# oscarkey/safe-exploration

Hardware: AMD Instinct MI355X
Metric: cem_particle_step_evals_per_s (higher is better)
Workload: dtype f64

## Files before the change

### include/sx_amd.h

```cpp
#ifndef SX_AMD_H
#define SX_AMD_H

#include <stdint.h>

#ifdef __cplusplus
extern "C" {
#endif

#define SX_MAX_NS 4
#define SX_MAX_NU 2
#define SX_MAX_D (SX_MAX_NS + SX_MAX_NU)
#define SX_MAX_M 16
#define SX_TILE 16

#define SX_OK 0
#define SX_ERR_ARG 1
#define SX_ERR_UNSUPPORTED 2
#define SX_ERR_LAUNCH 3

#define SX_STATUS_NAN 1
#define SX_STATUS_ZERO_FIX 2
#define SX_STATUS_UB_NONPOS 4

#define SX_OBJ_NEG_VARIANCE 0
#define SX_OBJ_AFFINE_ABS 1
#define SX_CON_TERMINAL 0
#define SX_CON_ALL_STATES 1

#define SX_ACTION_VIOLATION_COST 3.0
#define SX_STATE_VIOLATION_COST 10.0

typedef struct sx_gp_model {
    int32_t n_s, n_u;
    int32_t n_train;
    int32_t n_pad;
    double inv_ls2[SX_MAX_NS * SX_MAX_D];
    double outputscale[SX_MAX_NS];
    double noise[SX_MAX_NS];
    const double* x_train;
    const double* a_pack;
    const int32_t* stage_tab;
} sx_gp_model;

typedef struct sx_env {
    int32_t n_s, n_u;
    int32_t m;
    int32_t obj_mode;
    int32_t con_mode;
    int32_t reserved;
    double beta;
    double a[SX_MAX_NS * SX_MAX_NS];
    double b[SX_MAX_NS * SX_MAX_NU];
    double k_fb[SX_MAX_NU * SX_MAX_NS];
    double l_mu[SX_MAX_NS];
    double l_sigma[SX_MAX_NS];
    double h_mat[SX_MAX_M * SX_MAX_NS];
    double h_vec[SX_MAX_M];
    double u_min[SX_MAX_NU];
    double u_max[SX_MAX_NU];
    double obj_w_abs[SX_MAX_NS];
    double obj_target[SX_MAX_NS];
    double obj_w_lin[SX_MAX_NS];
} sx_env;

const char* sx_version(void);

#define SX_FEAT_MAX_WIDTH 32
#define SX_FEAT_MAX_LAYERS 3
typedef struct sx_feat_model {
    int32_t n_s, n_u;
    int32_t n_feat;
    int32_t n_layers;
    int32_t normalise;
    int32_t width[SX_FEAT_MAX_LAYERS + 1];
    double prelu;
// ... 174 lines not shown
```

### safe_exploration_amd/csrc/sx_rollout_rh.hpp

```cpp
#pragma once
#include <hip/hip_runtime.h>

#include "../../include/sx_amd.h"
#include "sx_rollout_rw.hpp"

#ifndef SX_RH_REGP
#define SX_RH_REGP 26
#endif
#ifndef SX_RH_LEAD
#define SX_RH_LEAD -1
#endif
#ifndef SX_RH_LDSP
#define SX_RH_LDSP 8
#endif
#ifndef SX_RH_PFG
#define SX_RH_PFG 6
#endif
#ifndef SX_RH_PFL
#define SX_RH_PFL 2
#endif
#ifndef SX_RH_RBMAJOR
#define SX_RH_RBMAJOR 1
#endif
#ifndef SX_RH_PRIO
#define SX_RH_PRIO 0
#endif
#ifndef SX_RH_WFIRST
#define SX_RH_WFIRST 0
#endif
#ifndef SX_RH_SHARES
#define SX_RH_SHARES 4, 4, 4, 1, 4, 4, 4
#endif

namespace sx {

constexpr int kRhWaves = 8;
constexpr int kRhThreads = 64 * kRhWaves;

template <int NS, int NRB>
struct RhPlan {
    int wave_of[NS][NRB];
    int pairs[kRhWaves];
    constexpr RhPlan() : wave_of{}, pairs{} {
        for (int w = 0; w < kRhWaves; ++w) pairs[w] = 0;
        for (int d = 0; d < NS; ++d) {
            int lo = 0, n = kRhWaves;
            if (kRhWaves % NS == 0) {
                n = kRhWaves / NS;
                lo = d * n;
            }
            const bool rev = (kRhWaves % NS == 0) && (d & 1);
            int set_of[NRB] = {};
            int load[kRhWaves] = {};
            for (int rb = NRB - 1; rb >= 0; --rb) {
                int best = 0;
                for (int s = 1; s < n; ++s)
                    if (load[s] + pairs[lo + (rev ? n - 1 - s : s)] < load[best] + pairs[lo + (rev ? n - 1 - best : best)]) best = s;
                set_of[rb] = best;
                load[best] += 2 * (rb + 1);
            }
            for (int rb = 0; rb < NRB; ++rb) wave_of[d][rb] = lo + (rev ? n - 1 - set_of[rb] : set_of[rb]);
            for (int s = 0; s < n; ++s) pairs[lo + (rev ? n - 1 - s : s)] += load[s];
        }
    }
    constexpr int max_pairs() const {
        int m = 0;
        for (int w = 0; w < kRhWaves; ++w) m = pairs[w] > m ? pairs[w] : m;
        return m;
    }
    constexpr bool has(int w, int d) const {
        for (int rb = 0; rb < NRB; ++rb)
            if (wave_of[d][rb] == w) return true;
        return false;
    }
    constexpr int qmax(int w, int d) const {
        for (int rb = NRB - 1; rb >= 0; --rb)
            if (wave_of[d][rb] == w) return 2 * (rb + 1);
        return 0;
    }
};

template <int NS, int NRB>
struct RhElements {
    static constexpr int kMax = NS * NRB * (NRB + 1);
    short d[kRhWaves][kMax], rb[kRhWaves][kMax], q[kRhWaves][kMax];
    int n[kRhWaves];
    constexpr RhElements() : d{}, rb{}, q{}, n{} {
        const RhPlan<NS, NRB> plan{};
        for (int w = 0; w < kRhWaves; ++w) {
            int idx = 0;
            for (int dd = 0; dd < NS; ++dd) {
#if SX_RH_RBMAJOR
                for (int r = NRB - 1; r >= 0; --r)
                    for (int qq = 0; qq < 2 * (r + 1); ++qq)
                        if (plan.wave_of[dd][r] == w) { d[w][idx] = dd; rb[w][idx] = r; q[w][idx] = qq; ++idx; }
#else
                for (int qq = 0; qq < 2 * NRB; ++qq)
                    for (int r = NRB - 1; r >= 0; --r)
                        if (plan.wave_of[dd][r] == w && qq < 2 * (r + 1)) { d[w][idx] = dd; rb[w][idx] = r; q[w][idx] = qq; ++idx; }
#endif
            }
            n[w] = idx;
        }
    }
};

struct RhLayout {
    int nr, nl, ng, lead;
    constexpr RhLayout(int total, int regp, int ldsp)
        : nr(total < regp ? total : regp), nl(0), ng(0), lead(0) {
        nl = total - nr < ldsp ? total - nr : ldsp;
        ng = total - nr - nl;
        lead = SX_RH_LEAD < 0 || ng == 0 ? nr : (SX_RH_LEAD < nr ? SX_RH_LEAD : nr);
    }
    constexpr int storage(int e, int regp, int ldsp) const {
        if (SX_RH_LEAD < 0 || ng == 0) return e;
        if (e < lead) return e;
        if (e < lead + ng) return regp + ldsp + (e - lead);
        if (e < lead + ng + nl) return regp + (e - lead - ng);
        return lead + (e - lead - ng - nl);
    }
};

template <int NS, int NRB, int MAXP, int REGP, int LDSP>
struct RhStream {
    int pair[kRhWaves][MAXP];
    constexpr RhStream() : pair{} {
        const RhElements<NS, NRB> el{};
        constexpr int wpo = NRB * (NRB + 1);
        for (int w = 0; w < kRhWaves; ++w) {
            const RhLayout lay(el.n[w], REGP, LDSP);
            for (int i = 0; i < MAXP; ++i) pair[w][i] = 0;
            for (int e = 0; e < el.n[w]; ++e)
                pair[w][lay.storage(e, REGP, LDSP)] = el.d[w][e] * wpo + el.rb[w][e] * (el.rb[w][e] + 1) + el.q[w][e];
        }
    }
};

enum RhOpKind { kRhLoadB = 0, kRhLoadWL = 1, kRhLoadWG = 2, kRhMfma = 3, kRhRowEpi = 4, kRhFinalEpi = 5 };
struct RhOp {
    int kind;
    int i;
    int rb;
    int q;
    int d;
    int slot;
    int e;
};
template <int NS, int NRB, int WAVE, int REGP, int LDSP, int PF, int PFL, int PFG>
struct RhProgram {
    static constexpr int kMaxOps = 4 * NS * NRB * (NRB + 1) / 2 + 8 * NRB * NS + 16;
    RhOp ops[kMaxOps];
    int n;
    int total;
    constexpr RhProgram() : ops{}, n(0), total(0) {
        const RhElements<NS, NRB> el{};
        total = el.n[WAVE];
        const RhLayout lay(total, REGP, LDSP);
        int next_l = 0;
        int next_g = 0;
        const int e_g0 = (SX_RH_LEAD < 0 || lay.ng == 0) ? lay.nr + lay.nl : lay.lead;
        const int e_l0 = (SX_RH_LEAD < 0 || lay.ng == 0) ? lay.nr : lay.lead + lay.ng;
        int bslot[RhElements<NS, NRB>::kMax] = {};
        int bfirst[RhElements<NS, NRB>::kMax] = {};
        int nloads = 0;
        for (int e = 0; e < total; ++e) {
            const bool fresh = SX_RH_RBMAJOR || e == 0 || el.q[WAVE][e] != el.q[WAVE][e - 1] || el.d[WAVE][e] != el.d[WAVE][e - 1];
            if (fresh) ++nloads;
            bfirst[e] = fresh ? 1 : 0;
            bslot[e] = (nloads - 1) % (PF + 1);
        }
        constexpr int kDelay = 2;
        int pend_rb[NRB * NS] = {}, pend_d[NRB * NS] = {}, pend_at[NRB * NS] = {};
        int npend = 0, done = 0;
        int issued_b = 0;
        int eb = 0;
        auto issue_b_upto = [&](int loads_wanted) {
            while (issued_b < loads_wanted && eb < total) {
                if (bfirst[eb]) {
                    ops[n++] = RhOp{kRhLoadB, 0, 0, el.q[WAVE][eb], el.d[WAVE][eb], bslot[eb]};
                    ++issued_b;
                }
                ++eb;
            }
        };
        int loads_seen = 0;
        for (int e = 0; e < total; ++e) {
            if (bfirst[e]) ++loads_seen;
            issue_b_upto(loads_seen + PF);
            while (next_l < lay.nl && e_l0 + next_l <= e + PFL) ops[n++] = RhOp{kRhLoadWL, REGP + next_l++, 0, 0, 0, 0};
            while (next_g < lay.ng && e_g0 + next_g <= e + PFG) ops[n++] = RhOp{kRhLoadWG, REGP + LDSP + next_g++, 0, 0, 0, 0};
            ops[n++] = RhOp{kRhMfma, lay.storage(e, REGP, LDSP), el.rb[WAVE][e], el.q[WAVE][e], el.d[WAVE][e], bslot[e], e};
            const bool last_of_rb = el.q[WAVE][e] == 2 * (el.rb[WAVE][e] + 1) - 1;
            if (last_of_rb) {
                pend_rb[npend] = el.rb[WAVE][e];
                pend_d[npend] = el.d[WAVE][e];
                pend_at[npend] = e + kDelay;
                ++npend;
            }
            while (done < npend && pend_at[done] <= e) {
                ops[n++] = RhOp{kRhRowEpi, 0, pend_rb[done], 0, pend_d[done], 0};
                ++done;
            }
        }
        while (done < npend) {
            ops[n++] = RhOp{kRhRowEpi, 0, pend_rb[done], 0, pend_d[done], 0};
            ++done;
        }
        const RhPlan<NS, NRB> plan{};
        for (int d = 0; d < NS; ++d)
            if (plan.has(WAVE, d)) ops[n++] = RhOp{kRhFinalEpi, 0, 0, 0, d, 0};
    }
};

template <int NS, int D, int NRB, int WAVE, int REGP, int LDSP>
__device__ __forceinline__ void rh_mfma_phase(const GpConst<NS, D>& gc, GpTileLds<NS, D>& lds, const v2d* wlds_wave, int lane,
                                              const v2d (&wreg)[REGP]) {
    constexpr int PF = SX_RW_PF, PFL = SX_RH_PFL, PFG = SX_RH_PFG;
    constexpr int MAXP = RhPlan<NS, NRB>{}.max_pairs();
    static constexpr RhProgram<NS, NRB, WAVE, REGP, LDSP, PF, PFL, PFG> prog{};
    static constexpr RhStream<NS, NRB, MAXP, REGP, LDSP> stream{};
    const v2d* kbase = reinterpret_cast<const v2d*>(lds.kfrag) + lane;
    typedef const __attribute__((address_space(1))) v2d* gv2d;
    typedef const __attribute__((address_space(3))) v2d* lv2d;
    const v2d* ap_opaque = reinterpret_cast<const v2d*>(gc.a_pack) + lane;
    asm volatile("" : "+v"(ap_opaque));
    const gv2d ap = (gv2d)ap_opaque;
    const lv2d wl_base = (lv2d)wlds_wave + lane;
    v4d acc[NRB];
    v2d b[PF + 1];
    v2d wl[PFL + 1];
    v2d wg[PFG + 1];
    double ssq[NS];
#pragma unroll
    for (int d = 0; d < NS; ++d) ssq[d] = 0.0;
    static_for<0, prog.n>([&](auto ktag) {
        constexpr RhOp op = prog.ops[decltype(ktag)::value];
        if constexpr (op.kind == kRhLoadB) {
            b[op.slot] = kbase[(op.q * NS + op.d) * 64];
        } else if constexpr (op.kind == kRhLoadWL) {
            wl[op.i % (PFL + 1)] = wl_base[(op.i - REGP) * 64];
        } else if constexpr (op.kind == kRhLoadWG) {
            wg[op.i % (PFG + 1)] = ap[(size_t)stream.pair[WAVE][op.i] * 64];
        } else if constexpr (op.kind == kRhMfma) {
#if SX_RH_PRIO == 2
            if constexpr ((4 * op.e) / prog.total != (4 * (op.e - 1)) / prog.total || op.e == 0)
                __builtin_amdgcn_s_setprio(3 - (4 * op.e) / prog.total);
#endif
            SX_PIN();
            const v2d bq = b[op.slot];
            v2d a;
            if constexpr (op.i < REGP)
                a = wreg[op.i];
            else if constexpr (op.i < REGP + LDSP)
                a = wl[op.i % (PFL + 1)];
            else
                a = wg[op.i % (PFG + 1)];
            if constexpr (op.q == 0)
                acc[op.rb] = __builtin_amdgcn_mfma_f64_16x16x4f64(a.x, bq.x, v4d{0.0, 0.0, 0.0, 0.0}, 0, 0, 0);
            else
                acc[op.rb] = __builtin_amdgcn_mfma_f64_16x16x4f64(a.x, bq.x, acc[op.rb], 0, 0, 0);
            acc[op.rb] = __builtin_amdgcn_mfma_f64_16x16x4f64(a.y, bq.y, acc[op.rb], 0, 0, 0);
            SX_PIN();
        } else if constexpr (op.kind == kRhRowEpi) {
            constexpr int rb = op.rb, d = op.d;
            double s;
            if constexpr (rb >= NRB - 2) {
                const int row0 = rb * 16 + (lane >> 4);
                s = 0.0;
#pragma unroll
                for (int r = 0; r < 4; ++r) {
                    const int row = row0 + 4 * r;
                    if (row < gc.n_train)
                        s = fma(acc[rb][r], acc[rb][r], s);
                    else if (row - gc.n_train <= D)
                        lds.mj[d * 256 + (row - gc.n_train) * 16 + (lane & 15)] = acc[rb][r];
                }
            } else {
                s = fma(acc[rb][3], acc[rb][3], fma(acc[rb][2], acc[rb][2], fma(acc[rb][1], acc[rb][1], acc[rb][0] * acc[rb][0])));
            }
            ssq[d] += s;
        } else {
            constexpr int d = op.d;
            const v4d tot = __builtin_amdgcn_mfma_f64_16x16x4f64(1.0, ssq[d], v4d{0.0, 0.0, 0.0, 0.0}, 0, 0, 0);
            if (lane < 16) lds.part[(WAVE * NS + d) * 16 + lane] = tot[0];
        }
    });
}

template <int NS, int D, int NRB, bool WITH_JAC, typename G>
__device__ __forceinline__ void rh_collect(const G& gc, const GpTileLds<NS, D>& lds, int c, const double (&z)[D],
                                           double (&mean)[NS], double (&var)[NS], double (&jac)[NS][D]) {
    constexpr RhPlan<NS, NRB> plan{};
#pragma unroll
    for (int d = 0; d < NS; ++d) {
        double q = 0.0;
#pragma unroll
        for (int w = 0; w < kRhWaves; ++w)
            if (plan.has(w, d)) q += lds.part[(w * NS + d) * 16 + c];
        var[d] = (gc.outputscale[d] - q) + gc.noise[d];
        const double m = lds.mj[d * 256 + c];
        mean[d] = m;
        if constexpr (WITH_JAC) {
#pragma unroll
            for (int j = 0; j < D; ++j) jac[d][j] = lds.mj[d * 256 + (1 + j) * 16 + c] - z[j] * gc.inv_ls2[d * D + j] * m;
        }
    }
}

template <int NS, int NRB>
constexpr int rh_regp() {
    constexpr int m = RhPlan<NS, NRB>{}.max_pairs();
    return m < SX_RH_REGP ? m : SX_RH_REGP;
}
template <int NS, int NRB>
constexpr int rh_ldsp() {
    constexpr int rest = RhPlan<NS, NRB>{}.max_pairs() - rh_regp<NS, NRB>();
    return rest < SX_RH_LDSP ? rest : SX_RH_LDSP;
}
template <int NS, int NU, int NRB>
inline size_t rh_lds_doubles(int n_train, int n_pad, int H) {
    constexpr int D = NS + NU, S = NS + NS * NS;
    return (size_t)NS * n_pad * 16 + NS * 256 + (size_t)kRhWaves * NS * 16 + 32 * D + (((size_t)SX_TILE * H * NU + 1) & ~(size_t)1) +
           (((size_t)SX_TILE * (2 * (S + NS) + 3) + 1) & ~(size_t)1) + RwKstarLds<NS, D>::doubles(n_pad) +
           (size_t)kRhWaves * rh_ldsp<NS, NRB>() * 128;
}

template <int NS, int NU, int NRB>
__global__ __launch_bounds__(kRhThreads) void cem_rollout_rh_kernel(GpConst<NS, NS + NU> gc, ReachConst<NS, NU> rc,
                                                                    CostConst<SX_MAX_M, NS, NU> cc, RolloutPtrs rp) {
    constexpr int D = NS + NU;
    constexpr int S = NS + NS * NS;
    constexpr int PQS = S + NS;
    constexpr RhPlan<NS, NRB> plan{};
    constexpr int MAXP = plan.max_pairs();
    constexpr int REGP = rh_regp<NS, NRB>();
    constexpr int LDSP = rh_ldsp<NS, NRB>();
    extern __shared__ __attribute__((aligned(16))) double smem[];
    GpTileLds<NS, D> lds;
    constexpr int nw = kRhWaves;
    lds.xs = nullptr;
    lds.etab = nullptr;
    lds.kfrag = smem;
    lds.mj = lds.kfrag + (size_t)NS * gc.n_pad * 16;
    lds.part = lds.mj + NS * 256;
    lds.zs = lds.part + (size_t)nw * NS * 16;
    double* acts = lds.zs + 32 * D;
    const int tid = threadIdx.x;
    const int wave = __builtin_amdgcn_readfirstlane(tid >> 6), lane = tid & 63;
    const int H = rp.H;
    const int tiles_per_problem = (rp.P + SX_TILE - 1) / SX_TILE;
    const int total_tiles = rp.E * tiles_per_problem;

    RwConst<NS, NU>* const cst = reinterpret_cast<RwConst<NS, NU>*>(acts + (((size_t)SX_TILE * rp.H * NU + 1) & ~(size_t)1));
    double* const pq = reinterpret_cast<double*>(cst + 1);
    RwKstarLds<NS, D> kl;
    kl.carve(pq + (((size_t)SX_TILE * (2 * PQS + 3) + 1) & ~(size_t)1), gc.n_pad);
    v2d* const wlds = reinterpret_cast<v2d*>(kl.xbar + ((D + 1) & ~1));

    static constexpr RhStream<NS, NRB, MAXP, REGP, LDSP> stream{};
    v2d wreg[REGP];
#if SX_RH_WFIRST
    {
        const v2d* __restrict__ const ap0 = reinterpret_cast<const v2d*>(gc.a_pack) + lane;
#pragma unroll
        for (int i = 0; i < REGP; ++i) wreg[i] = ap0[(size_t)stream.pair[wave][i] * 64];
        if constexpr (LDSP > 0) {
#pragma unroll
            for (int i = 0; i < LDSP; ++i) wlds[(wave * LDSP + i) * 64 + lane] = ap0[(size_t)stream.pair[wave][REGP + i] * 64];
        }
    }
#endif
    {
        static_assert(sizeof(RwConst<NS, NU>) % 8 == 0 && sizeof(ReachConst<NS, NU>) % 8 == 0 &&
                      sizeof(CostConst<SX_MAX_M, NS, NU>) % 8 == 0, "copied in 8-byte words");
        constexpr int nrc = sizeof(ReachConst<NS, NU>) / 8, ncc = sizeof(CostConst<SX_MAX_M, NS, NU>) / 8;
        double* dst = reinterpret_cast<double*>(cst);
        const double* src_rc = reinterpret_cast<const double*>(&rc);
        const double* src_cc = reinterpret_cast<const double*>(&cc);
        for (int i = tid; i < nrc; i += kRhThreads) dst[i] = src_rc[i];
        for (int i = tid; i < ncc; i += kRhThreads) dst[nrc + i] = src_cc[i];
        if (tid < NS * D) cst->inv_ls2[tid] = gc.inv_ls2[tid];
        if (tid < NS) {
            cst->outputscale[tid] = gc.outputscale[tid];
            cst->noise[tid] = gc.noise[tid];
        }
    }
    const RwConst<NS, NU>& fc = *cst;
    const ReachConst<NS, NU>& frc = cst->rc;
    const CostConst<SX_MAX_M, NS, NU>& fcc = cst->cc;
    rw_kstar_setup(gc, kl, lds.kfrag);
    const int kstar_pairs = (gc.n_train + 7) >> 3;

    const bool owner = tid < SX_TILE;
    int q0_begin, q0_end, q_begin = 0, q_end = 0;
    kstar_pair_range(kstar_pairs, wave, 1, nw, q0_begin, q0_end);
    if (wave > 0) {
        constexpr int kShare[8] = {0, SX_RH_SHARES};
        int before = 0, total = 0;
#pragma unroll
        for (int w = 1; w < 8; ++w) {
            if (w < wave) before += kShare[w];
            total += kShare[w];
        }
        kstar_pair_range(kstar_pairs, before, kShare[wave], total, q_begin, q_end);
    }
    double* const zs_base = lds.zs;

    for (int tile = blockIdx.x; tile < total_tiles; tile += gridDim.x) {
#ifdef SX_STAMPS
        const unsigned long long tile_t0 = stamp();
        unsigned long long first_k = 0, first_kb = 0;
#endif
        const int e = tile / tiles_per_problem;
        const int c0 = (tile - e * tiles_per_problem) * SX_TILE;
        const bool valid = owner && (c0 + tid < rp.P);

        const double* dist_mean = rp.mean + (int64_t)e * H * NU;
        const double* dist_std = rp.std + (int64_t)e * H * NU;
        bool have_q = rp.q0 != nullptr;
        if (rp.elite_rows) {
            const int L = H * NU, W = 2 + L;
            double* const ms = lds.kfrag;
            const double* rows = rp.elite_rows + (int64_t)e * rp.elite_k * W + 2;
            const bool publish = c0 == 0 && rp.mean_out;
// ... 8 lines not shown
                    ms[col] = m;
                    ms[L + col] = sd;
                    if (publish) {
                        rp.mean_out[(int64_t)e * L + col] = m;
                        rp.std_out[(int64_t)e * L + col] = sd;
                    }
                }
            }
            __syncthreads();
            dist_mean = ms;
            dist_std = ms + L;
        }
        for (int i = tid; i < SX_TILE * H * NU; i += kRhThreads) {
            const int c = i / (H * NU);
            const int r = i - c * (H * NU);
            double a = 0.0;
            if (c0 + c < rp.P) {
                const int64_t gi = ((int64_t)e * rp.P + c0 + c) * (H * NU) + r;
                if (rp.noise) {
                    a = dist_mean[r] + dist_std[r] * rp.noise[gi];
                    rp.actions[gi] = a;
                } else {
                    a = rp.actions[gi];
                }
            }
            acts[i] = a;
        }
        const bool lane_owner = lane < SX_TILE;
        const bool lane_valid = lane_owner && (c0 + lane < rp.P);
        auto st_row = [&](int buf, int c) { return pq + (buf * SX_TILE + c) * PQS; };
        double* const ac_row = pq + 2 * SX_TILE * PQS + (lane_owner ? lane : 0) * 3;
        if (owner) {
            double* my = st_row(0, tid);
#pragma unroll
            for (int i = 0; i < NS; ++i) {
                my[i] = rp.x0[(int64_t)e * NS + i];
#pragma unroll
                for (int j = 0; j < NS; ++j) my[NS + i * NS + j] = have_q ? rp.q0[((int64_t)e * NS + i) * NS + j] : 0.0;
            }
            ac_row[0] = 0.0;
            ac_row[1] = 0.0;
            reinterpret_cast<int*>(ac_row + 2)[0] = 0;
        }
        __syncthreads();
        if (owner) {
            const double* my = st_row(0, tid);
#pragma unroll
            for (int i = 0; i < NS; ++i) lds.zs[tid * D + i] = my[i];
#pragma unroll
            for (int cidx = 0; cidx < NU; ++cidx) lds.zs[tid * D + NS + cidx] = acts[(tid * H + 0) * NU + cidx];
        }
        __syncthreads();

        if (!SX_RH_WFIRST && tile == (int)blockIdx.x) {
            const v2d* __restrict__ const ap = reinterpret_cast<const v2d*>(gc.a_pack) + lane;
            if constexpr (LDSP > 0) {
                const __amdgpu_buffer_rsrc_t arsrc =
                    __builtin_amdgcn_make_buffer_rsrc(const_cast<double*>(gc.a_pack), 0, (int)0xffffffffu, 0x00020000);
#pragma unroll
                for (int i = 0; i < LDSP; ++i) {
                    const int pair = __builtin_amdgcn_readfirstlane(stream.pair[wave][REGP + i]);
                    __builtin_amdgcn_raw_ptr_buffer_load_lds(
                        arsrc, (__attribute__((address_space(3))) void*)(wlds + (wave * LDSP + i) * 64), 16, lane * 16, pair << 10, 0, 0);
                }
            }
#pragma unroll
            for (int i = 0; i < REGP; ++i) wreg[i] = ap[(size_t)stream.pair[wave][i] * 64];
        }

        auto next_centre = [&](const ReachConst<NS, NU>& R, int c, const double* z_prev, double (&out)[NS]) {
#pragma unroll
            for (int i = 0; i < NS; ++i) {
                double s = lds.mj[i * 256 + c];
#pragma unroll
                for (int j = 0; j < NS; ++j) s = fma(R.a[i * NS + j], z_prev[j], s);
#pragma unroll
                for (int cidx = 0; cidx < NU; ++cidx) s = fma(R.b[i * NU + cidx], z_prev[NS + cidx], s);
                out[i] = s;
            }
        };
        auto finish_state = [&](int t) {
            double z[D], u[NU], mean[NS], var[NS], jac[NS][D], p1[NS], Q1[NS][NS];
            double p[NS], Q[NS][NS];
            constexpr RhPlan<NS, NRB> plan{};
            const double* my = st_row(t & 1, lane);
            double partv[NS][kRhWaves], mjv[NS][1 + D], ils2[NS][D], osc[NS], nzv[NS];
#pragma unroll
            for (int d = 0; d < NS; ++d) {
#pragma unroll
                for (int w = 0; w < kRhWaves; ++w) partv[d][w] = plan.has(w, d) ? lds.part[(w * NS + d) * 16 + lane] : 0.0;
#pragma unroll
                for (int r = 0; r < 1 + D; ++r) mjv[d][r] = lds.mj[d * 256 + r * 16 + lane];
            }
#pragma unroll
            for (int i = 0; i < NS; ++i) {
                p[i] = my[i];
#pragma unroll
                for (int j = 0; j < NS; ++j) Q[i][j] = my[NS + i * NS + j];
            }
#pragma unroll
            for (int cidx = 0; cidx < NU; ++cidx) u[cidx] = acts[(lane * H + t) * NU + cidx];
#pragma unroll
            for (int d = 0; d < NS; ++d) {
                osc[d] = fc.outputscale[d];
                nzv[d] = fc.noise[d];
#pragma unroll
                for (int j = 0; j < D; ++j) ils2[d][j] = fc.inv_ls2[d * D + j];
// ... 101 lines not shown
                    }
                    const double dist = hc + sqrt(hq) - hv;
                    viol = viol || (dist >= 0.0);
                }
            }
            unsigned long long bits = __ballot(viol);
            bits |= bits >> 32;
            bits |= bits >> 16;
            if (lane_owner) {
                if ((bits >> lane) & 1ull) con += SX_STATE_VIOLATION_COST;
                bool uviol = false;
#pragma unroll
                for (int cidx = 0; cidx < NU; ++cidx) uviol = uviol || (uu[cidx] < umin[cidx]) || (uu[cidx] > umax[cidx]);
                if (uviol) con += SX_ACTION_VIOLATION_COST;
                double oadd = 0.0;
                if (obj_mode == SX_OBJ_NEG_VARIANCE) {
#pragma unroll
                    for (int i = 0; i < NS; ++i) oadd -= var[i];
                } else {
#pragma unroll
                    for (int i = 0; i < NS; ++i) oadd += wab[i] * fabs(tgt[i] - pp[i]) + wli[i] * pp[i];
                }
                obj += oadd;
                ac_row[0] = obj;
                ac_row[1] = con;
                const int64_t g = (int64_t)e * rp.P + c0 + lane;
                if (lane_valid && rp.traj) {
                    double* tr = rp.traj + (g * H + t) * S;
#pragma unroll
                    for (int i = 0; i < NS; ++i) {
                        tr[i] = pp[i];
#pragma unroll
                        for (int j = 0; j < NS; ++j) tr[NS + i * NS + j] = QQ[i][j];
                    }
                }
                if (lane_valid && rp.sigma) {
#pragma unroll
                    for (int i = 0; i < NS; ++i) rp.sigma[(g * H + t) * NS + i] = var[i];
                }
            }
        };

#ifdef SX_STAMPS
        unsigned long long c_k = 0, c_kb = 0, c_m = 0, c_mb = 0;
        unsigned long long rt0;
        asm volatile("s_memrealtime %0\n\ts_waitcnt lgkmcnt(0)" : "=s"(rt0)::"memory");
        const unsigned long long ct0 = stamp();
#endif
        for (int t = 0; t < H; ++t) {
#ifdef SX_STAMPS
            const unsigned long long t0 = stamp();
#endif
            const bool kstar_wave = !(t > 0 && wave == 0);
            if (wave == 4 && t > 1) finish_costs(t - 2);
            if (kstar_wave) {
                double zq[D];
                const int c = lane & 15;
                if (t == 0) {
#pragma unroll
                    for (int j = 0; j < D; ++j) zq[j] = zs_base[c * D + j];
                    rw_kstar_phase(gc, kl, lds.kfrag, q0_begin, q0_end, zq);
                } else {
                    double pc[NS];
                    next_centre(rc, c, zs_base + ((t - 1) & 1) * 16 * D + c * D, pc);
#pragma unroll
                    for (int i = 0; i < NS; ++i) zq[i] = pc[i];
#pragma unroll
                    for (int cidx = 0; cidx < NU; ++cidx) zq[NS + cidx] = acts[(c * H + t) * NU + cidx];
                    rw_kstar_phase(gc, kl, lds.kfrag, q_begin, q_end, zq);
                }
            } else if (owner) {
                finish_state(t - 1);
            }
#ifdef SX_STAMPS
            const unsigned long long t1 = stamp();
#endif
            if (t == 0) asm volatile("s_waitcnt vmcnt(0)" ::: "memory");
            __syncthreads();
#ifdef SX_STAMPS
            const unsigned long long t2 = stamp();
#endif
            const v2d* wl = wlds + wave * LDSP * 64;
#if SX_RH_PRIO == 1
            if (wave < 4) __builtin_amdgcn_s_setprio(3);
#endif
            switch (wave) {
                case 0: rh_mfma_phase<NS, D, NRB, 0, REGP, LDSP>(gc, lds, wl, lane, wreg); break;
                case 1: rh_mfma_phase<NS, D, NRB, 1, REGP, LDSP>(gc, lds, wl, lane, wreg); break;
                case 2: rh_mfma_phase<NS, D, NRB, 2, REGP, LDSP>(gc, lds, wl, lane, wreg); break;
                case 3: rh_mfma_phase<NS, D, NRB, 3, REGP, LDSP>(gc, lds, wl, lane, wreg); break;
                case 4: rh_mfma_phase<NS, D, NRB, 4, REGP, LDSP>(gc, lds, wl, lane, wreg); break;
                case 5: rh_mfma_phase<NS, D, NRB, 5, REGP, LDSP>(gc, lds, wl, lane, wreg); break;
                case 6: rh_mfma_phase<NS, D, NRB, 6, REGP, LDSP>(gc, lds, wl, lane, wreg); break;
                default: rh_mfma_phase<NS, D, NRB, 7, REGP, LDSP>(gc, lds, wl, lane, wreg); break;
            }
#if SX_RH_PRIO == 1
            if (wave < 4) __builtin_amdgcn_s_setprio(0);
#elif SX_RH_PRIO == 2
            __builtin_amdgcn_s_setprio(0);
#endif
#ifdef SX_STAMPS
            const unsigned long long t3 = stamp();
#endif
            __syncthreads();
#ifdef SX_STAMPS
            const unsigned long long t4 = stamp();
            c_k += t1 - t0; c_kb += t2 - t1; c_m += t3 - t2; c_mb += t4 - t3;
            if (t == 0) { first_k = t1 - t0; first_kb = t2 - t1; }
#endif
        }
#ifdef SX_STAMPS
        const unsigned long long loop_t1 = stamp();
        if (rp.stamps && lane == 0 && tile == (int)blockIdx.x) {
            unsigned long long* o = rp.stamps + ((size_t)blockIdx.x * nw + wave) * 8;
            o[0] = c_k; o[1] = c_kb; o[2] = c_m; o[3] = c_mb;
            o[4] = (ct0 - tile_t0) | (first_k << 32);
            unsigned long long rt1;
            asm volatile("s_memrealtime %0\n\ts_waitcnt lgkmcnt(0)" : "=s"(rt1)::"memory");
            o[6] = stamp() - ct0;
            o[7] = rt1 - rt0;
        }
#endif
        if (wave == 0 && owner) finish_state(H - 1);
        if (wave == 4 && H > 1) finish_costs(H - 2);
        __syncthreads();
        if (wave == 0) finish_costs(H - 1);
        if (valid) {
            const int64_t g = (int64_t)e * rp.P + c0 + tid;
            rp.obj_cost[g] = ac_row[0];
            rp.con_cost[g] = ac_row[1];
            const int st = reinterpret_cast<const int*>(ac_row + 2)[0];
            if (st) atomicOr(rp.status, st);
        }
        __syncthreads();
#ifdef SX_STAMPS
        if (rp.stamps && lane == 0 && tile == (int)blockIdx.x)
            rp.stamps[((size_t)blockIdx.x * nw + wave) * 8 + 5] = (stamp() - loop_t1) | (first_kb << 32);
#endif
    }
}

}
```

### safe_exploration_amd/csrc/sx_rollout_rw.hpp

```cpp
#pragma once
#include <hip/hip_runtime.h>

#include "../../include/sx_amd.h"
#include "sx_exp2_tab2048.hpp"
#include "sx_gp.hpp"
#include "sx_reach.hpp"
#include "sx_refit.hpp"
#include "sx_rollout.hpp"
#include "sx_rw_launch.hpp"

#ifndef SX_RW_LDSCONST
#define SX_RW_LDSCONST 1
#endif
#ifndef SX_RW_POLYLANES
#define SX_RW_POLYLANES 1
#endif
#ifndef SX_RW_PF
#define SX_RW_PF 2
#endif
#ifndef SX_RW_RCLOCAL
#define SX_RW_RCLOCAL 0
#endif
#ifndef SX_RW_POLYFOLD
#define SX_RW_POLYFOLD 0
// ... 146 lines not shown
        if (lane < 16) lds.part[(WAVE * NS + d) * 16 + lane] = tot[0];
        }
    });
}

constexpr double kExpScale2 = 2048.0 / 0.693147180559945309417232;
constexpr double kExpUnit2 = 0.693147180559945309417232 / 2048.0;

template <int NS, int D>
struct RwKstarLds {
    double* rows;
    double* tab;
    double* xbar;
    static __host__ __device__ size_t doubles(int n_pad) { return (size_t)n_pad * (D + NS) + (n_pad & 1) + kExpTab2 + 2 + ((D + 1) & ~1); }
    __device__ void carve(double* base, int n_pad) {
        rows = base;
        tab = rows + (size_t)n_pad * (D + NS) + (n_pad & 1);
        xbar = tab + kExpTab2 + 2;
    }
};

template <int NS, int D>
__device__ __forceinline__ void rw_kstar_setup(const GpConst<NS, D>& gc, const RwKstarLds<NS, D>& kl, double* kfrag) {
    const int tid = threadIdx.x, lane = tid & 63;
    double xb[D];
#pragma unroll
    for (int j = 0; j < D; ++j) {
        double v = lane < gc.n_train ? gc.x_train[lane * D + j] : 0.0;
        for (int off = 32; off > 0; off >>= 1) v += __shfl_xor(v, off);
        xb[j] = v / (double)(gc.n_train < 64 ? gc.n_train : 64);
        if (tid == 0) kl.xbar[j] = xb[j];
    }
    for (int k = tid; k < gc.n_pad; k += blockDim.x) {
        double xr[D], cc[NS];
#pragma unroll
        for (int d = 0; d < NS; ++d) cc[d] = 0.0;
#pragma unroll
        for (int j = 0; j < D; ++j) {
            xr[j] = k < gc.n_train ? gc.x_train[k * D + j] - xb[j] : 0.0;
#pragma unroll
            for (int d = 0; d < NS; ++d) cc[d] = fma(gc.k_nh_ils2[d * D + j], xr[j] * xr[j], cc[d]);
        }
#pragma unroll
        for (int j = 0; j < D; ++j) kl.rows[k * (D + NS) + j] = xr[j];
#pragma unroll
        for (int d = 0; d < NS; ++d) kl.rows[k * (D + NS) + D + d] = cc[d];
    }
    for (int i = tid; i < kExpTab2; i += blockDim.x) kl.tab[i] = kExp2Tab2048[i];
    if (tid < 2) kl.tab[kExpTab2 + tid] = __builtin_nan("");
    const int first_pad = ((gc.n_train + 7) >> 3) * NS * 128;
    for (int i = first_pad + tid; i < (gc.n_pad >> 3) * NS * 128; i += blockDim.x) kfrag[i] = 0.0;
}

template <int NS, int D>
__device__ __forceinline__ void rw_kstar_phase(const GpConst<NS, D>& gc, const RwKstarLds<NS, D>& kl, double* kfrag,
                                               int q_begin, int q_end, const double (&z)[D]) {
    constexpr int M = 2 * NS, RS = D + NS;
    const int n = q_end - q_begin;
    if (n <= 0) return;
    const int lane = (int)threadIdx.x & 63;
    const int c = lane & 15;
    double zz[NS], g[NS][D];
    bool znan = false;
    {
        double zc[D];
#pragma unroll
        for (int j = 0; j < D; ++j) {
            zc[j] = z[j] - kl.xbar[j];
            znan = znan || (z[j] != z[j]);
        }
#pragma unroll
        for (int d = 0; d < NS; ++d) {
            double a = gc.k_log_os[d];
#pragma unroll
            for (int j = 0; j < D; ++j) {
                const double kz = gc.k_nh_ils2[d * D + j] * zc[j];
                a = fma(kz, zc[j], a);
                g[d][j] = -2.0 * kz;
            }
            zz[d] = a;
        }
    }
    const lds_f64* etab = (const lds_f64*)kl.tab + (znan ? kExpTab2 : 0);
    const int emask = znan ? 0 : kExpTab2 - 1;
    const int k0 = 8 * q_begin + (lane >> 4);
    const lds_f64* x = (const lds_f64*)kl.rows + k0 * RS;
    lds_f64* f = (lds_f64*)kfrag + kfrag_index(NS, c, k0, 0);

    struct Set {
        double t[M], p[M];
        int mi[M];
    };
    auto load_x = [&](double (&xx)[2 * RS]) {
        asm volatile("" : "+v"(x));
#pragma unroll
        for (int h = 0; h < 2; ++h)
#pragma unroll
            for (int j = 0; j < RS; ++j) xx[h * RS + j] = x[h * 4 * RS + j];
        x += 8 * RS;
    };
    auto stage_a1 = [&](const double (&xx)[2 * RS], Set& s) {
        double yc[M], m[M];
#pragma unroll
        for (int h = 0; h < 2; ++h)
#pragma unroll
            for (int d = 0; d < NS; ++d) {
                double a = xx[h * RS + D + d] + zz[d];
#pragma unroll
                for (int j = 0; j < D; ++j) a = fma(g[d][j], xx[h * RS + j], a);
                yc[h * NS + d] = a;
            }
#pragma unroll
        for (int i = 0; i < M; ++i) yc[i] = __builtin_fmax(yc[i], -800.0 * kExpScale2);
#pragma unroll
        for (int i = 0; i < M; ++i) m[i] = __builtin_rint(yc[i]);
#pragma unroll
        for (int i = 0; i < M; ++i) asm("v_cvt_i32_f64 %0, %1" : "=v"(s.mi[i]) : "v"(m[i]));
#pragma unroll
        for (int i = 0; i < M; ++i) s.t[i] = etab[s.mi[i] & emask];
#pragma unroll
#if SX_RW_POLYFOLD
        for (int i = 0; i < M; ++i) s.p[i] = yc[i] - m[i];
#else
        for (int i = 0; i < M; ++i) s.p[i] = (yc[i] - m[i]) * kExpUnit2;
#endif
    };
    auto stage_a2 = [&](Set& s) {
        double r[M];
#pragma unroll
        for (int i = 0; i < M; ++i) r[i] = s.p[i];
#pragma unroll
#if SX_RW_POLYFOLD
        for (int i = 0; i < M; ++i) s.p[i] = fma(r[i], kExpUnit2 * kExpUnit2 * kExpUnit2 / 6.0, kExpUnit2 * kExpUnit2 * 0.5);
#pragma unroll
        for (int i = 0; i < M; ++i) s.p[i] = fma(s.p[i], r[i], kExpUnit2);
#else
        for (int i = 0; i < M; ++i) s.p[i] = fma(r[i], 1.66666666666666666667e-01, 0.5);
#pragma unroll
        for (int i = 0; i < M; ++i) s.p[i] = fma(s.p[i], r[i], 1.0);
#endif
#pragma unroll
        for (int i = 0; i < M; ++i) s.p[i] = s.p[i] * r[i];
    };
    auto stage_b = [&](const Set& s) {
        asm volatile("" : "+v"(f));
        double val[M];
#pragma unroll
        for (int i = 0; i < M; ++i) val[i] = ldexp(fma(s.t[i], s.p[i], s.t[i]), s.mi[i] >> 11);
#pragma unroll
        for (int d = 0; d < NS; ++d) {
            f[d * 128] = val[d];
            f[d * 128 + 1] = val[NS + d];
        }
        f += NS * 128;
    };
    double xr[2 * RS];
    Set s0, s1;
    load_x(xr);
    stage_a1(xr, s0);
    load_x(xr);
    stage_a2(s0);
    auto body = [&](const Set& sold, Set& snew) {
        stage_a1(xr, snew);
        SX_PIN();
        load_x(xr);
        stage_b(sold);
        SX_PIN();
        stage_a2(snew);
        SX_PIN();
    };
    const int n1 = n - 1;
    for (int k = 0; k < (n1 >> 1); ++k) {
        body(s0, s1);
        body(s1, s0);
    }
    if (n1 & 1) {
        body(s0, s1);
        stage_b(s1);
    } else {
        stage_b(s0);
    }
}

template <int NS, int NU>
struct alignas(16) RwConst {
    ReachConst<NS, NU> rc;
    CostConst<SX_MAX_M, NS, NU> cc;
    double inv_ls2[NS * (NS + NU)];
    double outputscale[NS];
    double noise[NS];
};

template <int NS, int D, int NRB, bool WITH_JAC, typename G>
__device__ __forceinline__ void rw_collect(const G& gc, const GpTileLds<NS, D>& lds, int c,
                                           const double (&z)[D], double (&mean)[NS], double (&var)[NS],
                                           double (&jac)[NS][D]) {
    constexpr RwPlan<NS, NRB> plan{};
#pragma unroll
    for (int d = 0; d < NS; ++d) {
        double q = 0.0;
#pragma unroll
        for (int w = 0; w < kRwWaves; ++w)
            if (plan.has(w, d)) q += lds.part[(w * NS + d) * 16 + c];
        var[d] = (gc.outputscale[d] - q) + gc.noise[d];
        const double m = lds.mj[d * 256 + c];
        mean[d] = m;
        if constexpr (WITH_JAC) {
#pragma unroll
            for (int j = 0; j < D; ++j) jac[d][j] = lds.mj[d * 256 + (1 + j) * 16 + c] - z[j] * gc.inv_ls2[d * D + j] * m;
        }
    }
}

template <int NS, int NU, int NRB>
__global__ __launch_bounds__(kRwThreads) __attribute__((amdgpu_waves_per_eu(1, 1)))
void cem_rollout_rw_kernel(GpConst<NS, NS + NU> gc, ReachConst<NS, NU> rc, CostConst<SX_MAX_M, NS, NU> cc, RolloutPtrs rp) {
    constexpr int D = NS + NU;
    constexpr int S = NS + NS * NS;
    constexpr int PQS = S + 3;
    constexpr RwPlan<NS, NRB> plan{};
    constexpr int MAXP = plan.max_pairs();
    static_assert(MAXP <= kRwMaxPairs, "W does not fit the register budget");
    extern __shared__ __attribute__((aligned(16))) double smem[];
    GpTileLds<NS, D> lds;
    constexpr int nw = kRwWaves;
    double* acts = lds.carve(smem, gc.n_train, gc.n_pad, nw, NS);
    const int tid = threadIdx.x;
#if SX_RW_LDSCONST
    RwConst<NS, NU>* const cst = reinterpret_cast<RwConst<NS, NU>*>(acts + (((size_t)SX_TILE * rp.H * NU + 1) & ~(size_t)1));
    {
        static_assert(sizeof(RwConst<NS, NU>) % 8 == 0 && sizeof(ReachConst<NS, NU>) % 8 == 0 &&
                      sizeof(CostConst<SX_MAX_M, NS, NU>) % 8 == 0, "copied in 8-byte words");
        constexpr int nrc = sizeof(ReachConst<NS, NU>) / 8, ncc = sizeof(CostConst<SX_MAX_M, NS, NU>) / 8;
        double* dst = reinterpret_cast<double*>(cst);
// ... 331 lines not shown
```

Measured before the change: 465.3 million.

## Replace block barrier with LDS generation-flag handoff between Kstar and MFMA waves

Result: slower. 429.8 million (-7.6%).

```diff
diff --git a/include/sx_amd.h b/include/sx_amd.h
--- a/include/sx_amd.h
+++ b/include/sx_amd.h
@@ -21,6 +21,7 @@
 #define SX_STATUS_NAN 1
 #define SX_STATUS_ZERO_FIX 2
 #define SX_STATUS_UB_NONPOS 4
+#define SX_STATUS_HANDOFF_TIMEOUT 32
 
 #define SX_OBJ_NEG_VARIANCE 0
 #define SX_OBJ_AFFINE_ABS 1
diff --git a/safe_exploration_amd/csrc/sx_rollout_rh.hpp b/safe_exploration_amd/csrc/sx_rollout_rh.hpp
--- a/safe_exploration_amd/csrc/sx_rollout_rh.hpp
+++ b/safe_exploration_amd/csrc/sx_rollout_rh.hpp
@@ -4,12 +4,6 @@
 #include "../../include/sx_amd.h"
 #include "sx_rollout_rw.hpp"
 
-#ifndef SX_RH_REGP
-#define SX_RH_REGP 26
-#endif
-#ifndef SX_RH_LEAD
-#define SX_RH_LEAD -1
-#endif
 #ifndef SX_RH_LDSP
 #define SX_RH_LDSP 8
 #endif
@@ -19,14 +13,17 @@
 #ifndef SX_RH_PFL
 #define SX_RH_PFL 2
 #endif
-#ifndef SX_RH_RBMAJOR
-#define SX_RH_RBMAJOR 1
-#endif
-#ifndef SX_RH_PRIO
-#define SX_RH_PRIO 0
-#endif
-#ifndef SX_RH_WFIRST
-#define SX_RH_WFIRST 0
+#ifndef SX_RH_HANDOFF
+#define SX_RH_HANDOFF 1
+#endif
+#ifndef SX_RH_REGP
+#define SX_RH_REGP (SX_RH_HANDOFF ? 24 : 26)
+#endif
+#ifndef SX_RH_PUBLISH_PAIRS
+#define SX_RH_PUBLISH_PAIRS 0
+#endif
+#ifndef SX_RH_WAIT_PAIRS
+#define SX_RH_WAIT_PAIRS 2
 #endif
 #ifndef SX_RH_SHARES
 #define SX_RH_SHARES 4, 4, 4, 1, 4, 4, 4
@@ -89,36 +86,20 @@
         const RhPlan<NS, NRB> plan{};
         for (int w = 0; w < kRhWaves; ++w) {
             int idx = 0;
-            for (int dd = 0; dd < NS; ++dd) {
-#if SX_RH_RBMAJOR
+            for (int dd = 0; dd < NS; ++dd)
                 for (int r = NRB - 1; r >= 0; --r)
                     for (int qq = 0; qq < 2 * (r + 1); ++qq)
                         if (plan.wave_of[dd][r] == w) { d[w][idx] = dd; rb[w][idx] = r; q[w][idx] = qq; ++idx; }
-#else
-                for (int qq = 0; qq < 2 * NRB; ++qq)
-                    for (int r = NRB - 1; r >= 0; --r)
-                        if (plan.wave_of[dd][r] == w && qq < 2 * (r + 1)) { d[w][idx] = dd; rb[w][idx] = r; q[w][idx] = qq; ++idx; }
-#endif
-            }
             n[w] = idx;
         }
     }
 };
 
 struct RhLayout {
-    int nr, nl, ng, lead;
-    constexpr RhLayout(int total, int regp, int ldsp)
-        : nr(total < regp ? total : regp), nl(0), ng(0), lead(0) {
+    int nr, nl, ng;
+    constexpr RhLayout(int total, int regp, int ldsp) : nr(total < regp ? total : regp), nl(0), ng(0) {
         nl = total - nr < ldsp ? total - nr : ldsp;
         ng = total - nr - nl;
-        lead = SX_RH_LEAD < 0 || ng == 0 ? nr : (SX_RH_LEAD < nr ? SX_RH_LEAD : nr);
-    }
-    constexpr int storage(int e, int regp, int ldsp) const {
-        if (SX_RH_LEAD < 0 || ng == 0) return e;
-        if (e < lead) return e;
-        if (e < lead + ng) return regp + ldsp + (e - lead);
-        if (e < lead + ng + nl) return regp + (e - lead - ng);
-        return lead + (e - lead - ng - nl);
     }
 };
 
@@ -129,15 +110,45 @@
         const RhElements<NS, NRB> el{};
         constexpr int wpo = NRB * (NRB + 1);
         for (int w = 0; w < kRhWaves; ++w) {
-            const RhLayout lay(el.n[w], REGP, LDSP);
             for (int i = 0; i < MAXP; ++i) pair[w][i] = 0;
             for (int e = 0; e < el.n[w]; ++e)
-                pair[w][lay.storage(e, REGP, LDSP)] = el.d[w][e] * wpo + el.rb[w][e] * (el.rb[w][e] + 1) + el.q[w][e];
+                pair[w][e] = el.d[w][e] * wpo + el.rb[w][e] * (el.rb[w][e] + 1) + el.q[w][e];
         }
     }
 };
 
-enum RhOpKind { kRhLoadB = 0, kRhLoadWL = 1, kRhLoadWG = 2, kRhMfma = 3, kRhRowEpi = 4, kRhFinalEpi = 5 };
+typedef volatile __attribute__((address_space(3))) int rh_lds_word;
+constexpr int kRhHandoffWords = 64;
+constexpr int kRhWaveWord0 = kRhHandoffWords - kRhWaves;
+constexpr int kRhHandoffPolls = 1 << 15;
+struct RhHandoff {
+    rh_lds_word* words;
+    int gen;
+    int* status;
+};
+__device__ __forceinline__ unsigned long long rh_handoff_look(const RhHandoff& ho, int lane) {
+    const int v = ho.words[lane];
+    const unsigned long long m = __ballot(v == ho.gen);
+    asm volatile("" ::: "memory");
+    return m;
+}
+__device__ __forceinline__ unsigned long long rh_handoff_wait(const RhHandoff& ho, unsigned long long need, int lane) {
+    unsigned long long m = 0;
+    for (int look = 0; look < kRhHandoffPolls; ++look) {
+        __builtin_amdgcn_s_sleep(2);
+        m = rh_handoff_look(ho, lane);
+        if ((m & need) == need) return m;
+    }
+    if (lane == 0) atomicOr(ho.status, SX_STATUS_HANDOFF_TIMEOUT | SX_STATUS_NAN);
+    return ~0ull;
+}
+__device__ __forceinline__ void rh_handoff_publish(const RhHandoff& ho, int q_from, int q_to, bool done, int wave, int lane) {
+    asm volatile("s_waitcnt lgkmcnt(0)" ::: "memory");
+    const bool mine = lane == 63 && done;
+    if (lane < q_to - q_from || mine) ho.words[mine ? kRhWaveWord0 + wave : q_from + lane] = ho.gen;
+}
+
+enum RhOpKind { kRhLoadB = 0, kRhLoadWL = 1, kRhLoadWG = 2, kRhMfma = 3, kRhRowEpi = 4, kRhFinalEpi = 5, kRhWaitPairs = 6, kRhWaitWaves = 7 };
 struct RhOp {
     int kind;
     int i;
@@ -145,52 +156,52 @@
     int q;
     int d;
     int slot;
-    int e;
 };
 template <int NS, int NRB, int WAVE, int REGP, int LDSP, int PF, int PFL, int PFG>
 struct RhProgram {
-    static constexpr int kMaxOps = 4 * NS * NRB * (NRB + 1) / 2 + 8 * NRB * NS + 16;
+    static constexpr int kMaxOps = 4 * NS * NRB * (NRB + 1) / 2 + 8 * NRB * NS + 2 * NRB + 18;
     RhOp ops[kMaxOps];
     int n;
     int total;
     constexpr RhProgram() : ops{}, n(0), total(0) {
         const RhElements<NS, NRB> el{};
+        const RhPlan<NS, NRB> plan{};
         total = el.n[WAVE];
         const RhLayout lay(total, REGP, LDSP);
         int next_l = 0;
         int next_g = 0;
-        const int e_g0 = (SX_RH_LEAD < 0 || lay.ng == 0) ? lay.nr + lay.nl : lay.lead;
-        const int e_l0 = (SX_RH_LEAD < 0 || lay.ng == 0) ? lay.nr : lay.lead + lay.ng;
-        int bslot[RhElements<NS, NRB>::kMax] = {};
-        int bfirst[RhElements<NS, NRB>::kMax] = {};
-        int nloads = 0;
-        for (int e = 0; e < total; ++e) {
-            const bool fresh = SX_RH_RBMAJOR || e == 0 || el.q[WAVE][e] != el.q[WAVE][e - 1] || el.d[WAVE][e] != el.d[WAVE][e - 1];
-            if (fresh) ++nloads;
-            bfirst[e] = fresh ? 1 : 0;
-            bslot[e] = (nloads - 1) % (PF + 1);
-        }
         constexpr int kDelay = 2;
         int pend_rb[NRB * NS] = {}, pend_d[NRB * NS] = {}, pend_at[NRB * NS] = {};
         int npend = 0, done = 0;
-        int issued_b = 0;
         int eb = 0;
+        int known = 0, qneed = 0;
+        for (int d = 0; d < NS; ++d) qneed = plan.qmax(WAVE, d) > qneed ? plan.qmax(WAVE, d) : qneed;
+        bool waves_waited = false;
         auto issue_b_upto = [&](int loads_wanted) {
-            while (issued_b < loads_wanted && eb < total) {
-                if (bfirst[eb]) {
-                    ops[n++] = RhOp{kRhLoadB, 0, 0, el.q[WAVE][eb], el.d[WAVE][eb], bslot[eb]};
-                    ++issued_b;
-                }
+            while (eb < loads_wanted && eb < total) {
+                const int q = el.q[WAVE][eb];
+                if (SX_RH_HANDOFF && q >= known) {
+                    int hi = (q / SX_RH_WAIT_PAIRS + 1) * SX_RH_WAIT_PAIRS;
+                    hi = hi < qneed ? hi : qneed;
+                    ops[n++] = RhOp{kRhWaitPairs, known, 0, hi, 0, 0};
+                    known = hi;
+                }
+                ops[n++] = RhOp{kRhLoadB, 0, 0, q, el.d[WAVE][eb], eb % (PF + 1)};
                 ++eb;
             }
         };
-        int loads_seen = 0;
+        auto row_epi = [&](int k) {
+            if (SX_RH_HANDOFF && !waves_waited && pend_rb[k] >= NRB - 2) {
+                ops[n++] = RhOp{kRhWaitWaves, 0, 0, 0, 0, 0};
+                waves_waited = true;
+            }
+            ops[n++] = RhOp{kRhRowEpi, 0, pend_rb[k], 0, pend_d[k], 0};
+        };
         for (int e = 0; e < total; ++e) {
-            if (bfirst[e]) ++loads_seen;
-            issue_b_upto(loads_seen + PF);
-            while (next_l < lay.nl && e_l0 + next_l <= e + PFL) ops[n++] = RhOp{kRhLoadWL, REGP + next_l++, 0, 0, 0, 0};
-            while (next_g < lay.ng && e_g0 + next_g <= e + PFG) ops[n++] = RhOp{kRhLoadWG, REGP + LDSP + next_g++, 0, 0, 0, 0};
-            ops[n++] = RhOp{kRhMfma, lay.storage(e, REGP, LDSP), el.rb[WAVE][e], el.q[WAVE][e], el.d[WAVE][e], bslot[e], e};
+            issue_b_upto(e + 1 + PF);
+            while (next_l < lay.nl && lay.nr + next_l <= e + PFL) ops[n++] = RhOp{kRhLoadWL, REGP + next_l++, 0, 0, 0, 0};
+            while (next_g < lay.ng && lay.nr + lay.nl + next_g <= e + PFG) ops[n++] = RhOp{kRhLoadWG, REGP + LDSP + next_g++, 0, 0, 0, 0};
+            ops[n++] = RhOp{kRhMfma, e, el.rb[WAVE][e], el.q[WAVE][e], el.d[WAVE][e], e % (PF + 1)};
             const bool last_of_rb = el.q[WAVE][e] == 2 * (el.rb[WAVE][e] + 1) - 1;
             if (last_of_rb) {
                 pend_rb[npend] = el.rb[WAVE][e];
@@ -198,16 +209,10 @@
                 pend_at[npend] = e + kDelay;
                 ++npend;
             }
-            while (done < npend && pend_at[done] <= e) {
-                ops[n++] = RhOp{kRhRowEpi, 0, pend_rb[done], 0, pend_d[done], 0};
-                ++done;
-            }
-        }
-        while (done < npend) {
-            ops[n++] = RhOp{kRhRowEpi, 0, pend_rb[done], 0, pend_d[done], 0};
-            ++done;
-        }
-        const RhPlan<NS, NRB> plan{};
+            while (done < npend && pend_at[done] <= e) row_epi(done++);
+        }
+        while (done < npend) row_epi(done++);
+        if (SX_RH_HANDOFF && !waves_waited && total > 0) ops[n++] = RhOp{kRhWaitWaves, 0, 0, 0, 0, 0};
         for (int d = 0; d < NS; ++d)
             if (plan.has(WAVE, d)) ops[n++] = RhOp{kRhFinalEpi, 0, 0, 0, d, 0};
     }
@@ -215,7 +220,7 @@
 
 template <int NS, int D, int NRB, int WAVE, int REGP, int LDSP>
 __device__ __forceinline__ void rh_mfma_phase(const GpConst<NS, D>& gc, GpTileLds<NS, D>& lds, const v2d* wlds_wave, int lane,
-                                              const v2d (&wreg)[REGP]) {
+                                              const v2d (&wreg)[REGP], const RhHandoff& ho) {
     constexpr int PF = SX_RW_PF, PFL = SX_RH_PFL, PFG = SX_RH_PFG;
     constexpr int MAXP = RhPlan<NS, NRB>{}.max_pairs();
     static constexpr RhProgram<NS, NRB, WAVE, REGP, LDSP, PF, PFL, PFG> prog{};
@@ -234,19 +239,21 @@
     double ssq[NS];
 #pragma unroll
     for (int d = 0; d < NS; ++d) ssq[d] = 0.0;
+    unsigned long long ready = 0;
+    if constexpr (SX_RH_HANDOFF && prog.total > 0) ready = rh_handoff_look(ho, lane);
     static_for<0, prog.n>([&](auto ktag) {
         constexpr RhOp op = prog.ops[decltype(ktag)::value];
-        if constexpr (op.kind == kRhLoadB) {
+        if constexpr (op.kind == kRhWaitPairs || op.kind == kRhWaitWaves) {
+            constexpr unsigned long long bits = op.kind == kRhWaitWaves ? ((1ull << kRhWaves) - 1) << kRhWaveWord0
+                                                                        : ((1ull << op.q) - 1) & ~((1ull << op.i) - 1);
+            if ((ready & bits) != bits) ready = rh_handoff_wait(ho, bits, lane);
+        } else if constexpr (op.kind == kRhLoadB) {
             b[op.slot] = kbase[(op.q * NS + op.d) * 64];
         } else if constexpr (op.kind == kRhLoadWL) {
             wl[op.i % (PFL + 1)] = wl_base[(op.i - REGP) * 64];
         } else if constexpr (op.kind == kRhLoadWG) {
             wg[op.i % (PFG + 1)] = ap[(size_t)stream.pair[WAVE][op.i] * 64];
         } else if constexpr (op.kind == kRhMfma) {
-#if SX_RH_PRIO == 2
-            if constexpr ((4 * op.e) / prog.total != (4 * (op.e - 1)) / prog.total || op.e == 0)
-                __builtin_amdgcn_s_setprio(3 - (4 * op.e) / prog.total);
-#endif
             SX_PIN();
             const v2d bq = b[op.slot];
             v2d a;
@@ -323,7 +330,7 @@
     constexpr int D = NS + NU, S = NS + NS * NS;
     return (size_t)NS * n_pad * 16 + NS * 256 + (size_t)kRhWaves * NS * 16 + 32 * D + (((size_t)SX_TILE * H * NU + 1) & ~(size_t)1) +
            (((size_t)SX_TILE * (2 * (S + NS) + 3) + 1) & ~(size_t)1) + RwKstarLds<NS, D>::doubles(n_pad) +
-           (size_t)kRhWaves * rh_ldsp<NS, NRB>() * 128;
+           (size_t)kRhWaves * rh_ldsp<NS, NRB>() * 128 + kRhHandoffWords / 2;
 }
 
 template <int NS, int NU, int NRB>
@@ -336,6 +343,7 @@
     constexpr int MAXP = plan.max_pairs();
     constexpr int REGP = rh_regp<NS, NRB>();
     constexpr int LDSP = rh_ldsp<NS, NRB>();
+    static_assert(2 * NRB <= kRhWaveWord0, "one hand-off word per Kstar pair");
     extern __shared__ __attribute__((aligned(16))) double smem[];
     GpTileLds<NS, D> lds;
     constexpr int nw = kRhWaves;
@@ -357,20 +365,14 @@
     RwKstarLds<NS, D> kl;
     kl.carve(pq + (((size_t)SX_TILE * (2 * PQS + 3) + 1) & ~(size_t)1), gc.n_pad);
     v2d* const wlds = reinterpret_cast<v2d*>(kl.xbar + ((D + 1) & ~1));
+    RhHandoff ho;
+    ho.words = (rh_lds_word*)reinterpret_cast<int*>(wlds + kRhWaves * LDSP * 64);
+    ho.gen = 0;
+    ho.status = rp.status;
+    if (SX_RH_HANDOFF && tid < kRhHandoffWords) ho.words[tid] = 0;
 
     static constexpr RhStream<NS, NRB, MAXP, REGP, LDSP> stream{};
     v2d wreg[REGP];
-#if SX_RH_WFIRST
-    {
-        const v2d* __restrict__ const ap0 = reinterpret_cast<const v2d*>(gc.a_pack) + lane;
-#pragma unroll
-        for (int i = 0; i < REGP; ++i) wreg[i] = ap0[(size_t)stream.pair[wave][i] * 64];
-        if constexpr (LDSP > 0) {
-#pragma unroll
-            for (int i = 0; i < LDSP; ++i) wlds[(wave * LDSP + i) * 64 + lane] = ap0[(size_t)stream.pair[wave][REGP + i] * 64];
-        }
-    }
-#endif
     {
         static_assert(sizeof(RwConst<NS, NU>) % 8 == 0 && sizeof(ReachConst<NS, NU>) % 8 == 0 &&
                       sizeof(CostConst<SX_MAX_M, NS, NU>) % 8 == 0, "copied in 8-byte words");
@@ -485,7 +487,7 @@
         }
         __syncthreads();
 
-        if (!SX_RH_WFIRST && tile == (int)blockIdx.x) {
+        if (tile == (int)blockIdx.x) {
             const v2d* __restrict__ const ap = reinterpret_cast<const v2d*>(gc.a_pack) + lane;
             if constexpr (LDSP > 0) {
                 const __amdgpu_buffer_rsrc_t arsrc =
@@ -693,6 +695,14 @@
             const unsigned long long t0 = stamp();
 #endif
             const bool kstar_wave = !(t > 0 && wave == 0);
+            ++ho.gen;
+            int published = t == 0 ? q0_begin : q_begin;
+            auto stored_upto = [&](int q) {
+                if (SX_RH_HANDOFF && SX_RH_PUBLISH_PAIRS > 0 && q - published >= SX_RH_PUBLISH_PAIRS) {
+                    rh_handoff_publish(ho, published, q, false, wave, lane);
+                    published = q;
+                }
+            };
             if (wave == 4 && t > 1) finish_costs(t - 2);
             if (kstar_wave) {
                 double zq[D];
@@ -700,7 +710,7 @@
                 if (t == 0) {
 #pragma unroll
                     for (int j = 0; j < D; ++j) zq[j] = zs_base[c * D + j];
-                    rw_kstar_phase(gc, kl, lds.kfrag, q0_begin, q0_end, zq);
+                    rw_kstar_phase(gc, kl, lds.kfrag, q0_begin, q0_end, zq, stored_upto);
                 } else {
                     double pc[NS];
                     next_centre(rc, c, zs_base + ((t - 1) & 1) * 16 * D + c * D, pc);
@@ -708,7 +718,7 @@
                     for (int i = 0; i < NS; ++i) zq[i] = pc[i];
 #pragma unroll
                     for (int cidx = 0; cidx < NU; ++cidx) zq[NS + cidx] = acts[(c * H + t) * NU + cidx];
-                    rw_kstar_phase(gc, kl, lds.kfrag, q_begin, q_end, zq);
+                    rw_kstar_phase(gc, kl, lds.kfrag, q_begin, q_end, zq, stored_upto);
                 }
             } else if (owner) {
                 finish_state(t - 1);
@@ -717,29 +727,28 @@
             const unsigned long long t1 = stamp();
 #endif
             if (t == 0) asm volatile("s_waitcnt vmcnt(0)" ::: "memory");
+#if SX_RH_HANDOFF
+            {
+                const int share_end = wave == nw - 1 ? 2 * NRB : !kstar_wave ? published : (t == 0 ? q0_end : q_end);
+                rh_handoff_publish(ho, published, share_end, true, wave, lane);
+            }
+#else
             __syncthreads();
+#endif
 #ifdef SX_STAMPS
             const unsigned long long t2 = stamp();
 #endif
             const v2d* wl = wlds + wave * LDSP * 64;
-#if SX_RH_PRIO == 1
-            if (wave < 4) __builtin_amdgcn_s_setprio(3);
-#endif
             switch (wave) {
-                case 0: rh_mfma_phase<NS, D, NRB, 0, REGP, LDSP>(gc, lds, wl, lane, wreg); break;
-                case 1: rh_mfma_phase<NS, D, NRB, 1, REGP, LDSP>(gc, lds, wl, lane, wreg); break;
-                case 2: rh_mfma_phase<NS, D, NRB, 2, REGP, LDSP>(gc, lds, wl, lane, wreg); break;
-                case 3: rh_mfma_phase<NS, D, NRB, 3, REGP, LDSP>(gc, lds, wl, lane, wreg); break;
-                case 4: rh_mfma_phase<NS, D, NRB, 4, REGP, LDSP>(gc, lds, wl, lane, wreg); break;
-                case 5: rh_mfma_phase<NS, D, NRB, 5, REGP, LDSP>(gc, lds, wl, lane, wreg); break;
-                case 6: rh_mfma_phase<NS, D, NRB, 6, REGP, LDSP>(gc, lds, wl, lane, wreg); break;
-                default: rh_mfma_phase<NS, D, NRB, 7, REGP, LDSP>(gc, lds, wl, lane, wreg); break;
-            }
-#if SX_RH_PRIO == 1
-            if (wave < 4) __builtin_amdgcn_s_setprio(0);
-#elif SX_RH_PRIO == 2
-            __builtin_amdgcn_s_setprio(0);
-#endif
+                case 0: rh_mfma_phase<NS, D, NRB, 0, REGP, LDSP>(gc, lds, wl, lane, wreg, ho); break;
+                case 1: rh_mfma_phase<NS, D, NRB, 1, REGP, LDSP>(gc, lds, wl, lane, wreg, ho); break;
+                case 2: rh_mfma_phase<NS, D, NRB, 2, REGP, LDSP>(gc, lds, wl, lane, wreg, ho); break;
+                case 3: rh_mfma_phase<NS, D, NRB, 3, REGP, LDSP>(gc, lds, wl, lane, wreg, ho); break;
+                case 4: rh_mfma_phase<NS, D, NRB, 4, REGP, LDSP>(gc, lds, wl, lane, wreg, ho); break;
+                case 5: rh_mfma_phase<NS, D, NRB, 5, REGP, LDSP>(gc, lds, wl, lane, wreg, ho); break;
+                case 6: rh_mfma_phase<NS, D, NRB, 6, REGP, LDSP>(gc, lds, wl, lane, wreg, ho); break;
+                default: rh_mfma_phase<NS, D, NRB, 7, REGP, LDSP>(gc, lds, wl, lane, wreg, ho); break;
+            }
 #ifdef SX_STAMPS
             const unsigned long long t3 = stamp();
 #endif
diff --git a/safe_exploration_amd/csrc/sx_rollout_rw.hpp b/safe_exploration_amd/csrc/sx_rollout_rw.hpp
--- a/safe_exploration_amd/csrc/sx_rollout_rw.hpp
+++ b/safe_exploration_amd/csrc/sx_rollout_rw.hpp
@@ -222,9 +222,9 @@
     for (int i = first_pad + tid; i < (gc.n_pad >> 3) * NS * 128; i += blockDim.x) kfrag[i] = 0.0;
 }
 
-template <int NS, int D>
+template <int NS, int D, typename F>
 __device__ __forceinline__ void rw_kstar_phase(const GpConst<NS, D>& gc, const RwKstarLds<NS, D>& kl, double* kfrag,
-                                               int q_begin, int q_end, const double (&z)[D]) {
+                                               int q_begin, int q_end, const double (&z)[D], F&& stored_upto) {
     constexpr int M = 2 * NS, RS = D + NS;
     const int n = q_end - q_begin;
     if (n <= 0) return;
@@ -330,11 +330,13 @@
     stage_a1(xr, s0);
     load_x(xr);
     stage_a2(s0);
+    int q_stored = q_begin;
     auto body = [&](const Set& sold, Set& snew) {
         stage_a1(xr, snew);
         SX_PIN();
         load_x(xr);
         stage_b(sold);
+        stored_upto(++q_stored);
         SX_PIN();
         stage_a2(snew);
         SX_PIN();
@@ -350,6 +352,12 @@
     } else {
         stage_b(s0);
     }
+}
+
+template <int NS, int D>
+__device__ __forceinline__ void rw_kstar_phase(const GpConst<NS, D>& gc, const RwKstarLds<NS, D>& kl, double* kfrag,
+                                               int q_begin, int q_end, const double (&z)[D]) {
+    rw_kstar_phase(gc, kl, kfrag, q_begin, q_end, z, [](int) {});
 }
 
 template <int NS, int NU>
```
